# SensorsINI/v2e

Hardware: NVIDIA H100
Metric: Mevents/s (higher is better)
Workload: dtype fp16 tensor-core convs (fp32 accumulate) + f64 pixel state

## Files before the change

include/v2e_b200.h:

```cpp
#ifndef V2E_B200_H
#define V2E_B200_H

#include <stdint.h>

#ifdef __cplusplus
extern "C" {
#endif

typedef enum V2eStatus {
    V2E_OK = 0,
    V2E_E_INVALID = -1,
    V2E_E_CUDA = -2,
    V2E_E_CAPACITY = -3,
    V2E_E_ITER_CAP = -4,
    V2E_E_STATE = -5,
    V2E_E_UNSUPPORTED = -6,
    V2E_E_FALLBACK = -7
} V2eStatus;

typedef enum V2eFrameDtype { V2E_U8 = 0, V2E_F32 = 1, V2E_F64 = 2 } V2eFrameDtype;

const char *v2e_last_error(void);
int v2e_version(void);
int v2e_abi_info(int *version, int *emu_cfg_size, int *frame_info_size, int *unet_weights_size);
// ... 139 lines not shown
int v2e_conv2d_lrelu_sm100(const void *x1_dev, int C1, const void *x2_dev, int C2,
                           const void *wgt_dev, const float *bias_dev, int Cout_pad, int KH, int KW,
                           int N, int H, int W, void *out_dev, int out_cstride, int out_mode,
                           int co_real, float slope, void *stream);

enum {
    V2E_CONV_TILE_AUTO = -1,
    V2E_CONV_TILE_LEGACY = 0,
    V2E_CONV_TILE_256x128 = 1,
    V2E_CONV_TILE_128x256 = 2
};
int v2e_conv2d_lrelu_sm100_tile(const void *x1_dev, int C1, const void *x2_dev, int C2,
                                const void *wgt_dev, const float *bias_dev, int Cout_pad, int KH, int KW,
                                int N, int H, int W, void *out_dev, int out_cstride, int out_mode,
                                int co_real, float slope, int tile, void *stream);
int v2e_conv_pick_tile(int C1, int C2, int Cout_pad, int KH, int KW, int N, int H, int W, int n_sms);

int v2e_conv2d_lrelu_sm100_strip(const void *x1_dev, int C1, const void *x2_dev, int C2,
                                 const void *wgt_row_dev, const float *bias_dev, int Cout_pad, int KH,
                                 int KW, int N, int H, int W, void *out_dev, int out_cstride,
                                 int out_mode, int co_real, float slope, void *stream);
int v2e_conv_strip_pick_kc(int C1, int C2, int Cout_pad, int KH, int KW, int W);

enum {
    V2E_STRIP_CHAIN_AUTO = -1,
    V2E_STRIP_CHAIN_PAIRED = 0,
    V2E_STRIP_CHAIN_STACKED = 1
};
int v2e_conv2d_lrelu_sm100_strip_chain(const void *x1_dev, int C1, const void *x2_dev, int C2,
                                       const void *wgt_row_dev, const float *bias_dev, int Cout_pad, int KH,
// ... 97 lines not shown
```

v2e_b200/_lib.py:

```python
import ctypes
import os

from . import build as _build

_LIB = None


class V2eEmuCfg(ctypes.Structure):
    _fields_ = [
        ("width", ctypes.c_int32), ("height", ctypes.c_int32),
        ("per_pixel_thres", ctypes.c_int32), ("hdr", ctypes.c_int32),
        ("pos_thres_nominal", ctypes.c_double), ("neg_thres_nominal", ctypes.c_double),
        ("cutoff_hz", ctypes.c_double), ("leak_rate_hz", ctypes.c_double),
        ("leak_jitter_fraction", ctypes.c_double), ("refractory_period_s", ctypes.c_double),
        ("shot_noise_rate_hz", ctypes.c_double), ("shot_inten_factor", ctypes.c_double),
        ("rng_mode", ctypes.c_int32), ("iter_cap", ctypes.c_int32),
        ("seed", ctypes.c_uint64),
        ("csdvs", ctypes.c_int32), ("max_frames_per_step", ctypes.c_int32),
        ("cs_tau_p_s", ctypes.c_double), ("cs_tau_h_s", ctypes.c_double),
        ("scidvs", ctypes.c_int32), ("photoreceptor_noise", ctypes.c_int32),
        ("rng_pixel_offset", ctypes.c_uint32), ("full_frame_px", ctypes.c_uint32),
        ("own_row0", ctypes.c_int32), ("own_rows", ctypes.c_int32),
        ("cs_halo_rows", ctypes.c_int32), ("reserved1", ctypes.c_int32),
    ]
# ... 61 lines not shown
    "v2e_emu_cs_pack": (_i, [_vp, _vp]),
    "v2e_emu_cs_unpack_from": (_i, [_vp, _vp, _vp, _vp]),
    "v2e_emu_cs_send_dev": (_vp, [_vp]),
    "v2e_emu_cs_chunk": (_i, [_vp, _i, _i, _vp]),
    "v2e_emu_cs_max_dev": (_vp, [_vp]),
    "v2e_emu_cs_advance": (_i, [_vp, _i, _i, _vp]),
    "v2e_emu_cs_update": (_i, [_vp, _vp, _i, _vp, _vp, _vp]),
    "v2e_emu_phase_filter": (_i, [_vp, _d, _d, _u64, _i, _vp]),
    "v2e_emu_read_counts": (_i, [_vp, ctypes.POINTER(ctypes.c_int32), _vp, _i, _vp]),
    "v2e_emu_phase_shot": (_i, [_vp, _vp, _i, _d, _d, _vp, _u64, _vp]),
    "v2e_emu_phase_emit": (_i, [_vp, _d, _d, _vp, _u64, _vp]),
    "v2e_conv2d_lrelu_sm100": (_i, [_vp, _i, _vp, _i, _vp, _vp, _i, _i, _i, _i, _i, _i, _vp, _i, _i, _i,
                                    ctypes.c_float, _vp]),
    "v2e_conv2d_lrelu_sm100_tile": (_i, [_vp, _i, _vp, _i, _vp, _vp, _i, _i, _i, _i, _i, _i, _vp, _i, _i, _i,
                                         ctypes.c_float, _i, _vp]),
    "v2e_conv_pick_tile": (_i, [_i, _i, _i, _i, _i, _i, _i, _i, _i]),
    "v2e_conv2d_lrelu_sm100_strip": (_i, [_vp, _i, _vp, _i, _vp, _vp, _i, _i, _i, _i, _i, _i, _vp, _i, _i, _i,
                                          ctypes.c_float, _vp]),
    "v2e_conv_strip_pick_kc": (_i, [_i, _i, _i, _i, _i, _i]),
    "v2e_conv2d_lrelu_sm100_strip_chain": (_i, [_vp, _i, _vp, _i, _vp, _vp, _i, _i, _i, _i, _i, _i, _vp, _i, _i, _i,
                                                ctypes.c_float, _i, _vp]),
    "v2e_conv_strip_pick_chain": (_i, [_i, _i, _i, _i, _i, _i]),
    "v2e_conv2d_up2_lrelu_sm100": (_i, [_vp, _i, _vp, _vp, _vp, _i, _i, _i, _i, _vp, _i, ctypes.c_float, _vp]),
    "v2e_conv_up2_fold_weights": (_i, [_vp, _i, _i, _i, _i, _vp]),
    "v2e_conv_up2_supported_c": (_i, [_i, _i, _i]),
    "v2e_slomo_create": (_i, [_i, _i, _i, _vp, _vp, ctypes.POINTER(_vp)]),
    "v2e_slomo_destroy": (_i, [_vp]),
    "v2e_slomo_set_pairs": (_i, [_vp, _vp, _i, _vp]),
    "v2e_slomo_max_flow": (_i, [_vp, ctypes.POINTER(ctypes.c_float), _vp]),
    "v2e_slomo_interp": (_i, [_vp, _d, _vp, _vp, _vp]),
# ... 106 lines not shown
```

v2e_b200/csrc/conv_tc.cu:

```cuda
#include <cuda.h>
#include <cuda_fp16.h>
#include <cuda_runtime.h>
#include <math.h>
#include <stdint.h>
#include <stdio.h>
#include <string.h>
#include <vector>

#include "../../include/v2e_b200.h"
#include "common.cuh"
#include "tc_common.cuh"

namespace {

constexpr int kTileH = 8, kTileW = 16, kBM = kTileH * kTileW;
constexpr int kStages = 4;
constexpr int kConvThreads = 288;
constexpr int kProducerWarp = 8;
constexpr int kConsumerWarps = 8;

struct ConvParams {
    int N, H, W;
    int C1, C2;
    int KH, KW;
    int KC;
    int BN;
    int stages;
    int co_fast;
    int tiles_x, tiles_y;
    int n_tiles;
    int out_cstride;
    int out_mode;
    int co_real;
    float slope;
    const float *bias;
    void *out;
};

__device__ __forceinline__ uint8_t *align1024(uint8_t *p) { return (uint8_t *)(((uintptr_t)p + 1023) & ~(uintptr_t)1023); }

__device__ __forceinline__ float lrelu(float x, float slope) { return x > 0.f ? x : x * slope; }

template <int BN>
__device__ __forceinline__ void epilogue_row(const float (&d)[BN / 2], int i, bool inb, size_t pix, int lane,
                                             const float *bias, float slope, int out_mode, void *out, int cstride,
                                             int co0, __half2 (&h)[BN / 8]) {
#pragma unroll
    for (int j = 0; j < BN / 8; j++) {
        const int c = 8 * j + 2 * (lane & 3);
        const float x0 = lrelu(d[4 * j + 2 * i] + __ldg(bias + c), slope);
        const float x1 = lrelu(d[4 * j + 2 * i + 1] + __ldg(bias + c + 1), slope);
        h[j] = __floats2half2_rn(x0, x1);
        if (inb) {
            if (out_mode == 0) *(__half2 *)((__half *)out + pix * cstride + co0 + c) = h[j];
            else if (j == 0) *(float2 *)((float *)out + pix * 8 + c) = make_float2(x0, x1);
        }
// ... 1 lines not shown
}

template <int BN>
__global__ void __launch_bounds__(kConvThreads, 1)
conv_tc_kernel(const __grid_constant__ CUtensorMap tmA, const __grid_constant__ CUtensorMap tmA2,
               const __grid_constant__ CUtensorMap tmB, const ConvParams p) {
    extern __shared__ __align__(1024) uint8_t smem_raw[];
    uint8_t *smem = align1024(smem_raw);
    const uint32_t a_bytes = kBM * p.KC * 2;
    const uint32_t b_bytes_raw = BN * p.KC * 2;
    const uint32_t b_bytes = (b_bytes_raw + 1023) & ~1023u;
    const uint32_t stage_bytes = a_bytes + b_bytes;
    __shared__ __align__(8) uint64_t full_bar[kStages], empty_bar[kStages];

    const int warp = threadIdx.x >> 5, lane = threadIdx.x & 31;
    const int tile = p.co_fast ? blockIdx.y : blockIdx.x;
    const int tx = tile % p.tiles_x, ty = (tile / p.tiles_x) % p.tiles_y, n = tile / (p.tiles_x * p.tiles_y);
    const int x0 = tx * kTileW, y0 = ty * kTileH;
    const int n0 = (p.co_fast ? blockIdx.x : blockIdx.y) * BN;
    const int Ctot = p.C1 + p.C2;
    const int slabs = Ctot / p.KC;
    const int k_iters = p.KH * p.KW * slabs;

    if (threadIdx.x == 0) {
        for (int s = 0; s < kStages; s++) { mbar_init(&full_bar[s], 1); mbar_init(&empty_bar[s], kConsumerWarps); }
        fence_barrier_init();
    }
    if (warp == kProducerWarp && lane == 0) {
        prefetch_tmap(&tmA);
        if (p.C2) prefetch_tmap(&tmA2);
        prefetch_tmap(&tmB);
    }
    __syncthreads();

    if (warp == kProducerWarp) {
        if (lane == 0) {
            int stage = 0;
            uint32_t phase = 0;
            const int ph = p.KH / 2, pw = p.KW / 2;
            for (int tap = 0; tap < p.KH * p.KW; tap++) {
                const int r = tap / p.KW, s = tap % p.KW;
                for (int sl = 0; sl < slabs; sl++) {
                    mbar_wait(&empty_bar[stage], phase ^ 1);
                    uint8_t *sa = smem + stage * stage_bytes, *sb = sa + a_bytes;
                    mbar_expect_tx(&full_bar[stage], a_bytes + b_bytes_raw);
                    const int c = sl * p.KC;
                    if (c < p.C1) tma_load_4d(sa, &tmA, &full_bar[stage], c, x0 + s - pw, y0 + r - ph, n);
                    else tma_load_4d(sa, &tmA2, &full_bar[stage], c - p.C1, x0 + s - pw, y0 + r - ph, n);
                    tma_load_2d(sb, &tmB, &full_bar[stage], tap * Ctot + c, n0);
                    if (++stage == p.stages) { stage = 0; phase ^= 1; }
                }
            }
        }
    } else {
        const int g = warp >> 2;
        const uint64_t d0 = make_smem_desc(smem_u32(smem), swizzle_layout(p.KC), 8u * p.KC * 2u);
        const uint32_t stage16 = stage_bytes >> 4, a16 = a_bytes >> 4, half16 = (64u * p.KC * 2u) >> 4;
        const int ksteps = p.KC / 16;
        float acc[BN / 2];
#pragma unroll
        for (int i = 0; i < BN / 2; i++) acc[i] = 0.f;
        int stage = 0, prev = -1;
        uint32_t phase = 0;
        for (int it = 0; it < k_iters; it++) {
            mbar_wait(&full_bar[stage], phase);
            const uint32_t base = (uint32_t)stage * stage16;
            wgmma_fence();
            for (int j = 0; j < ksteps; j++)
                wgmma_f16<BN>(acc, desc_add(d0, base + (uint32_t)g * half16 + 2u * j), desc_add(d0, base + a16 + 2u * j),
                              (uint32_t)((it | j) != 0));
            wgmma_commit();
            wgmma_wait<1>();
            if (prev >= 0) { __syncwarp(); if (lane == 0) mbar_arrive(&empty_bar[prev]); }
            prev = stage;
            if (++stage == p.stages) { stage = 0; phase ^= 1; }
        }
        wgmma_wait<0>();
        wgmma_fence_regs(acc);
        __half2 hv[BN / 8];
#pragma unroll
        for (int i = 0; i < 2; i++) {
            const int m = 64 * g + 16 * (warp & 3) + (lane >> 2) + 8 * i;
            const int py = y0 + m / kTileW, px = x0 + m % kTileW;
            const bool inb = py < p.H && px < p.W;
            const size_t pix = ((size_t)n * p.H + py) * p.W + px;
            epilogue_row<BN>(acc, i, inb, pix, lane, p.bias + n0, p.slope, p.out_mode, p.out, p.out_cstride, n0, hv);
        }
    }
}

template <int MH, int BN>
__global__ void __launch_bounds__(kConvThreads, 1)
conv_wide_kernel(const __grid_constant__ CUtensorMap tmA, const __grid_constant__ CUtensorMap tmA2,
                 const __grid_constant__ CUtensorMap tmB, const ConvParams p) {
    constexpr int TH = kTileH * MH, BM = kBM * MH;
    extern __shared__ __align__(1024) uint8_t smem_raw[];
    uint8_t *smem = align1024(smem_raw);
    const uint32_t a_bytes = BM * p.KC * 2;
    const uint32_t b_bytes = BN * p.KC * 2;
    const uint32_t stage_bytes = a_bytes + b_bytes;
    __shared__ __align__(8) uint64_t full_bar[kStages], empty_bar[kStages];

    const int warp = threadIdx.x >> 5, lane = threadIdx.x & 31;
    const int tile = p.co_fast ? blockIdx.y : blockIdx.x;
    const int tx = tile % p.tiles_x, ty = (tile / p.tiles_x) % p.tiles_y, n = tile / (p.tiles_x * p.tiles_y);
    const int x0 = tx * kTileW, y0 = ty * TH;
    const int n0 = (p.co_fast ? blockIdx.x : blockIdx.y) * BN;
    const int Ctot = p.C1 + p.C2;
    const int slabs = Ctot / p.KC;
    const int k_iters = p.KH * p.KW * slabs;

    if (threadIdx.x == 0) {
        for (int s = 0; s < kStages; s++) { mbar_init(&full_bar[s], 1); mbar_init(&empty_bar[s], kConsumerWarps); }
        fence_barrier_init();
    }
    if (warp == kProducerWarp && lane == 0) {
        prefetch_tmap(&tmA);
        if (p.C2) prefetch_tmap(&tmA2);
        prefetch_tmap(&tmB);
    }
    __syncthreads();

    if (warp == kProducerWarp) {
        if (lane == 0) {
            int stage = 0;
            uint32_t phase = 0;
            const int ph = p.KH / 2, pw = p.KW / 2;
            for (int tap = 0; tap < p.KH * p.KW; tap++) {
                const int r = tap / p.KW, s = tap % p.KW;
                for (int sl = 0; sl < slabs; sl++) {
                    mbar_wait(&empty_bar[stage], phase ^ 1);
                    uint8_t *sa = smem + stage * stage_bytes, *sb = sa + a_bytes;
                    mbar_expect_tx(&full_bar[stage], a_bytes + b_bytes);
                    const int c = sl * p.KC;
                    if (c < p.C1) tma_load_4d(sa, &tmA, &full_bar[stage], c, x0 + s - pw, y0 + r - ph, n);
                    else tma_load_4d(sa, &tmA2, &full_bar[stage], c - p.C1, x0 + s - pw, y0 + r - ph, n);
                    tma_load_2d(sb, &tmB, &full_bar[stage], tap * Ctot + c, n0);
                    if (++stage == p.stages) { stage = 0; phase ^= 1; }
                }
            }
        }
    } else {
        const int g = __shfl_sync(0xffffffffu, warp >> 2, 0);
        const uint64_t d0 = make_smem_desc(smem_u32(smem), swizzle_layout(p.KC), 8u * p.KC * 2u);
        const uint32_t stage16 = stage_bytes >> 4, a16 = a_bytes >> 4, q16 = (64u * p.KC * 2u) >> 4;
        const int ksteps = p.KC / 16;
        float acc[MH][BN / 2];
#pragma unroll
        for (int h = 0; h < MH; h++) {
#pragma unroll
            for (int i = 0; i < BN / 2; i++) acc[h][i] = 0.f;
            wgmma_fence_regs(acc[h]);
        }
        int stage = 0, prev = -1;
        uint32_t phase = 0;
        for (int it = 0; it < k_iters; it++) {
            mbar_wait(&full_bar[stage], phase);
            const uint32_t base = (uint32_t)stage * stage16;
            wgmma_fence();
            for (int j = 0; j < ksteps; j++) {
#pragma unroll
                for (int h = 0; h < MH; h++)
                    wgmma_f16<BN>(acc[h], desc_add(d0, base + (uint32_t)(g * MH + h) * q16 + 2u * j),
                                  desc_add(d0, base + a16 + 2u * j), (uint32_t)((it | j) != 0));
            }
            wgmma_commit();
            wgmma_wait<1>();
            if (prev >= 0) { __syncwarp(); if (lane == 0) mbar_arrive(&empty_bar[prev]); }
            prev = stage;
            if (++stage == p.stages) { stage = 0; phase ^= 1; }
        }
        wgmma_wait<0>();
#pragma unroll
        for (int h = 0; h < MH; h++) wgmma_fence_regs(acc[h]);
        const float *bias = p.bias + n0;
        __half *out = (__half *)p.out + n0;
#pragma unroll
        for (int h = 0; h < MH; h++) {
            size_t pix[2];
            bool inb[2];
#pragma unroll
            for (int i = 0; i < 2; i++) {
                const int m = 64 * (g * MH + h) + 16 * (warp & 3) + (lane >> 2) + 8 * i;
                const int py = y0 + m / kTileW, px = x0 + m % kTileW;
                inb[i] = py < p.H && px < p.W;
                pix[i] = (((size_t)n * p.H + py) * p.W + px) * p.out_cstride;
            }
#pragma unroll
            for (int j = 0; j < BN / 8; j++) {
                const int c = 8 * j + 2 * (lane & 3);
                const float2 b = __ldg((const float2 *)(bias + c));
#pragma unroll
                for (int i = 0; i < 2; i++)
                    if (inb[i])
                        *(__half2 *)(out + pix[i] + c) = __floats2half2_rn(lrelu(acc[h][4 * j + 2 * i] + b.x, p.slope),
                                                                           lrelu(acc[h][4 * j + 2 * i + 1] + b.y, p.slope));
            }
        }
    }
}


constexpr int kRowTile = 128;

struct StripParams {
    int N, H, W;
    int C1, C2;
    int KH, KW;
    int KC, BN;
    int tiles_x, seg_h, n_seg, n_items;
    int nslot;
    void *pool_out;
// ... 528 lines not shown
        long tiles = (long)((W + kTileW - 1) / kTileW) * ((H + kTileH * mh - 1) / (kTileH * mh)) * N;
        const long ctas = tiles * (Cout_pad / bn);
        const long waves = (ctas + n_sms - 1) / n_sms;
        const double a_bytes = (double)kBM * mh * kc * 2, b_bytes = (double)bn * kc * 2;
        const double flops = 2.0 * kBM * mh * bn * kc;
        const double per_stage = fmax((a_bytes + b_bytes) / 24.0, flops / 4096.0);
        const double cost = (double)waves * per_stage;
        if (tile == V2E_CONV_TILE_LEGACY || cost < best_cost) { best = tile; best_cost = cost; }
    }
    return best;
}

struct V2eConvLaunch {
    CUtensorMap tmA, tmA2, tmB;
    ConvParams p;
    dim3 grid;
    int mh;
    size_t smem;
};

int v2e_conv_prepare(V2eConvLaunch *L, const void *x1, int C1, const void *x2, int C2, const void *wgt,
                     const float *bias, int Cout_pad, int KH, int KW, int N, int H, int W, void *out,
                     int out_cstride, int out_mode, int co_real, float slope, int tile, int n_sms) {
    if (C1 % 16 || C2 % 16 || !(Cout_pad == 16 || Cout_pad == 32 || Cout_pad == 64 || (Cout_pad > 0 && Cout_pad % 128 == 0)))
        return v2e_set_error(V2E_E_INVALID, "conv: channel counts must be padded to 16 (Cout to 16/32/64/128k)%s", "");
    if (tile == V2E_CONV_TILE_AUTO) tile = v2e_conv_pick_tile(C1, C2, Cout_pad, KH, KW, N, H, W, n_sms);
    if (tile < V2E_CONV_TILE_LEGACY || tile > V2E_CONV_TILE_128x256)
        return v2e_set_error(V2E_E_INVALID, "conv: unknown tile%s", "");
    memset(L, 0, sizeof(*L));
    ConvParams &p = L->p;
    int mh, bn;
    tile_shape(tile, Cout_pad, &mh, &bn);
    const bool wide = tile != V2E_CONV_TILE_LEGACY;
    p.N = N; p.H = H; p.W = W; p.C1 = C1; p.C2 = C2; p.KH = KH; p.KW = KW;
    p.KC = v2e_conv_pick_kc(C1, C2);
    p.BN = bn;
    if (wide && (Cout_pad % bn || out_mode != 0))
        return v2e_set_error(V2E_E_INVALID, "conv: the wide tiles need fp16 output and Cout_pad a multiple of their width%s", "");
    p.stages = kStages;
    p.tiles_x = (W + kTileW - 1) / kTileW;
    p.tiles_y = (H + kTileH * mh - 1) / (kTileH * mh);
    p.n_tiles = p.tiles_x * p.tiles_y * N;
    p.out_cstride = out_cstride; p.out_mode = out_mode; p.co_real = co_real; p.slope = slope;
    p.bias = bias; p.out = out;
    L->mh = mh;
    int rc;
    if ((rc = make_act_tmap_h(&L->tmA, x1, N, H, W, C1, p.KC, kTileH * mh))) return rc;
    if (C2) { if ((rc = make_act_tmap_h(&L->tmA2, x2, N, H, W, C2, p.KC, kTileH * mh))) return rc; }
    else L->tmA2 = L->tmA;
    if ((rc = v2e_make_wgt_tmap(&L->tmB, wgt, Cout_pad, KH * KW * (C1 + C2), p.KC, bn))) return rc;
    const unsigned tiles = (unsigned)p.n_tiles, cob = (unsigned)(Cout_pad / p.BN);
    p.co_fast = (cob > 1 && tiles <= 65535u) ? 1 : 0;
    L->grid = p.co_fast ? dim3(cob, tiles, 1) : dim3(tiles, cob, 1);
    size_t stage = (size_t)kBM * mh * p.KC * 2 + (((size_t)p.BN * p.KC * 2 + 1023) & ~(size_t)1023);
    L->smem = stage * p.stages + 1024;
    return V2E_OK;
}

template <int BN>
static cudaError_t conv_launch_bn(const V2eConvLaunch *L, cudaStream_t st) {
    static PerDeviceOnce attr_once;
    if (attr_once.first()) cudaFuncSetAttribute(conv_tc_kernel<BN>, cudaFuncAttributeMaxDynamicSharedMemorySize, 200 * 1024);
    conv_tc_kernel<BN><<<L->grid, kConvThreads, L->smem, st>>>(L->tmA, L->tmA2, L->tmB, L->p);
    return cudaGetLastError();
}

template <int MH, int BN>
static cudaError_t conv_launch_wide(const V2eConvLaunch *L, cudaStream_t st) {
    static PerDeviceOnce attr_once;
    if (attr_once.first())
        cudaFuncSetAttribute(conv_wide_kernel<MH, BN>, cudaFuncAttributeMaxDynamicSharedMemorySize, 226 * 1024);
    conv_wide_kernel<MH, BN><<<L->grid, kConvThreads, L->smem, st>>>(L->tmA, L->tmA2, L->tmB, L->p);
    return cudaGetLastError();
}

int v2e_conv_launch(const V2eConvLaunch *L, cudaStream_t st) {
    cudaError_t e;
    if (L->mh == 2 && L->p.BN == 128) e = conv_launch_wide<2, 128>(L, st);
    else if (L->mh == 1 && L->p.BN == 256) e = conv_launch_wide<1, 256>(L, st);
    else switch (L->p.BN) {
        case 16: e = conv_launch_bn<16>(L, st); break;
        case 32: e = conv_launch_bn<32>(L, st); break;
        case 64: e = conv_launch_bn<64>(L, st); break;
        case 128: e = conv_launch_bn<128>(L, st); break;
        default: return v2e_set_error(V2E_E_UNSUPPORTED, "conv_tc_kernel: unsupported tile width%s", "");
    }
    if (e != cudaSuccess) return v2e_set_error(V2E_E_CUDA, "conv_tc_kernel launch: %s", cudaGetErrorString(e));
    return V2E_OK;
}

size_t v2e_conv_launch_size(void) { return sizeof(V2eConvLaunch); }

static int device_sms() {
    int dev = 0, sms = 132;
    cudaGetDevice(&dev);
    cudaDeviceGetAttribute(&sms, cudaDevAttrMultiProcessorCount, dev);
    return sms;
}

extern "C" int v2e_conv2d_lrelu_sm100_tile(const void *x1_dev, int C1, const void *x2_dev, int C2,
                                           const void *wgt_dev, const float *bias_dev, int Cout_pad, int KH, int KW,
                                           int N, int H, int W, void *out_dev, int out_cstride, int out_mode,
                                           int co_real, float slope, int tile, void *stream) {
    V2eConvLaunch L;
    int rc = v2e_conv_prepare(&L, x1_dev, C1, x2_dev, C2, wgt_dev, bias_dev, Cout_pad, KH, KW, N, H, W, out_dev,
                              out_cstride, out_mode, co_real, slope, tile, device_sms());
    if (rc) return rc;
    return v2e_conv_launch(&L, (cudaStream_t)stream);
}

extern "C" int v2e_conv2d_lrelu_sm100(const void *x1_dev, int C1, const void *x2_dev, int C2,
                                      const void *wgt_dev, const float *bias_dev, int Cout_pad, int KH, int KW,
                                      int N, int H, int W, void *out_dev, int out_cstride, int out_mode,
                                      int co_real, float slope, void *stream) {
    return v2e_conv2d_lrelu_sm100_tile(x1_dev, C1, x2_dev, C2, wgt_dev, bias_dev, Cout_pad, KH, KW, N, H, W, out_dev,
                                       out_cstride, out_mode, co_real, slope, V2E_CONV_TILE_AUTO, stream);
}

struct V2eStripLaunch {
    CUtensorMap tmA, tmA2, tmB;
    StripParams p;
    int stacked;
    int grid;
// ... 344 lines not shown
```

v2e_b200/csrc/slomo.cu:

```cuda
#include <cuda.h>
#include <cuda_fp16.h>
#include <cuda_runtime.h>
#include <math.h>
#include <stdint.h>
#include <stdio.h>
#include <string.h>

#include <vector>

#include "../../include/v2e_b200.h"
#include "common.cuh"

struct V2eConvLaunch;
int v2e_conv_prepare(V2eConvLaunch *L, const void *x1, int C1, const void *x2, int C2, const void *wgt,
                     const float *bias, int Cout_pad, int KH, int KW, int N, int H, int W, void *out,
                     int out_cstride, int out_mode, int co_real, float slope, int tile, int n_sms);
int v2e_conv_launch(const V2eConvLaunch *L, cudaStream_t st);
size_t v2e_conv_launch_size(void);
struct V2eStripLaunch;
int v2e_strip_pick(int C1, int C2, int Cout_pad, int KH, int KW, int W, int *nslot_out);
size_t v2e_strip_launch_size(void);
int v2e_strip_pool_supported(int C1, int C2, int Cout_pad, int KH, int KW, int H, int W);
int v2e_strip_prepare(V2eStripLaunch *L, const void *x1, int C1, const void *x2, int C2, const void *wgt_row,
                      const float *bias, int Cout_pad, int KH, int KW, int N, int H, int W, void *out,
                      int out_cstride, int out_mode, int co_real, float slope, int n_sms, void *pool_out,
                      int pool_cstride, int chain);
int v2e_strip_launch(const V2eStripLaunch *L, cudaStream_t st);
struct V2eUpLaunch;
int v2e_conv_up2_supported(int C, int Cout_pad, int W_out);
extern "C" int v2e_conv_up2_fold_weights(const float *w, int cout, int cin, int Cout_pad, int C_pad, void *out_host);
size_t v2e_conv_up2_launch_size(void);
// ... 427 lines not shown
static int conv(V2eSlomo *h, const UNet &u, int li, const __half *x1, const __half *x2, int B, int H, int W, void *out,
                int out_mode, cudaStream_t st, __half *pool_out = nullptr) {
    int rc;
    const bool row = u.row_kc[li] != 0;
    V2eConvLaunch *L = (V2eConvLaunch *)h->launch_mem.data();
    V2eStripLaunch *R = (V2eStripLaunch *)h->row_mem.data();
    h->ran[&u == &h->interp][li] = row ? (pool_out ? V2E_SLOMO_KERNEL_STRIP_POOL : V2E_SLOMO_KERNEL_STRIP)
                                       : V2E_SLOMO_KERNEL_TAP;
    if (row)
        rc = v2e_strip_prepare(R, x1, u.c1p[li], x2, x2 ? u.c2p[li] : 0, u.w_row[li], u.b[li], u.cout_pad[li], u.L[li].k,
                               u.L[li].k, B, H, W, out, u.cout_pad[li], out_mode, u.L[li].cout, kSlope, h->n_sms,
                               pool_out, u.cout_pad[li], V2E_STRIP_CHAIN_AUTO);
    else
        rc = v2e_conv_prepare(L, x1, u.c1p[li], x2, x2 ? u.c2p[li] : 0, u.w[li], u.b[li], u.cout_pad[li], u.L[li].k,
                              u.L[li].k, B, H, W, out, u.cout_pad[li], out_mode, u.L[li].cout, kSlope,
                              V2E_CONV_TILE_AUTO, h->n_sms);
    if (rc) return rc;
    if (h->profile) {
        if (h->ev_used + 2 > h->ev.size()) {
            size_t old = h->ev.size();
            h->ev.resize(old + 512);
            for (size_t i = old; i < h->ev.size(); i++) cudaEventCreate(&h->ev[i]);
        }
        cudaEventRecord(h->ev[h->ev_used], st);
    }
    rc = row ? v2e_strip_launch(R, st) : v2e_conv_launch(L, st);
    if (h->profile) {
        cudaEventRecord(h->ev[h->ev_used + 1], st);
        h->ev_used += 2;
        const LayerSpec &l = u.L[li];
        const double fl = 2.0 * B * H * W * (double)l.cout * (l.cin1 + l.cin2) * l.k * l.k;
// ... 20 lines not shown
    }
    rc = v2e_conv_up2_launch(L, st);
    if (h->profile) {
        cudaEventRecord(h->ev[h->ev_used + 1], st);
        h->ev_used += 2;
        const LayerSpec &l = u.L[li];
        const double fl = 2.0 * B * H * W * (double)l.cout * l.cin1 * 9;
        h->conv_flops += fl;
        h->ev_layer.push_back(li);
        h->ev_flops.push_back(fl);
    }
    return rc;
}

static bool pool_fusable(const V2eSlomo *h, const UNet &u, int li, int H, int W) {
    if (h->no_fused_pool || !u.row_kc[li] || u.cout_pad[li] != u.L[li].cout) return false;
    return v2e_strip_pool_supported(u.c1p[li], u.c2p[li], u.cout_pad[li], u.L[li].k, u.L[li].k, H, W) != 0;
}

static int unet_forward(V2eSlomo *h, const UNet &u, const __half *in, float *out, int B, cudaStream_t st) {
    const int H = h->H, W = h->W;
    int rc;
    if ((rc = conv(h, u, 0, in, nullptr, B, H, W, h->x0, 0, st))) return rc;
    bool pooled = pool_fusable(h, u, 1, H, W);
    if ((rc = conv(h, u, 1, h->x0, nullptr, B, H, W, h->s1, 0, st, pooled ? h->pool[0] : nullptr))) return rc;
    const int ch[6] = {32, 64, 128, 256, 512, 512};
    const __half *prev = h->s1;
    for (int l = 0; l < 5; l++) {
        const int hi = H >> l, wi = W >> l, ho = hi / 2, wo = wi / 2;
        if (!pooled) {
            const long n = (long)B * ho * wo * (ch[l] / 8);
// ... 233 lines not shown
```

v2e_b200/csrc/tc_common.cuh:

```cuda
#pragma once
#include <cuda.h>
#include <cuda_runtime.h>
#include <stdint.h>

__device__ __forceinline__ uint32_t smem_u32(const void *p) { return (uint32_t)__cvta_generic_to_shared(p); }

__device__ __forceinline__ void mbar_init(uint64_t *bar, uint32_t count) {
    asm volatile("mbarrier.init.shared::cta.b64 [%0], %1;" ::"r"(smem_u32(bar)), "r"(count) : "memory");
}
__device__ __forceinline__ void fence_barrier_init() { asm volatile("fence.mbarrier_init.release.cluster;" ::: "memory"); }
__device__ __forceinline__ void fence_proxy_async() { asm volatile("fence.proxy.async.shared::cta;" ::: "memory"); }
__device__ __forceinline__ void mbar_expect_tx(uint64_t *bar, uint32_t bytes) {
    asm volatile("mbarrier.arrive.expect_tx.shared::cta.b64 _, [%0], %1;" ::"r"(smem_u32(bar)), "r"(bytes) : "memory");
}
__device__ __forceinline__ void mbar_arrive(uint64_t *bar) {
    asm volatile("mbarrier.arrive.shared::cta.b64 _, [%0];" ::"r"(smem_u32(bar)) : "memory");
}
__device__ __forceinline__ void mbar_wait(uint64_t *bar, uint32_t parity) {
    const uint32_t addr = smem_u32(bar);
    uint32_t done;
    do {
        asm volatile(
            "{\n\t.reg .pred p;\n\t"
            "mbarrier.try_wait.parity.shared::cta.b64 p, [%1], %2;\n\t"
// ... 3 lines not shown
}

__device__ __forceinline__ void prefetch_tmap(const CUtensorMap *tm) {
    asm volatile("prefetch.tensormap [%0];" ::"l"((uint64_t)tm) : "memory");
}
__device__ __forceinline__ void tma_load_4d(void *dst, const CUtensorMap *tm, uint64_t *bar, int c0, int c1, int c2, int c3) {
    asm volatile(
        "cp.async.bulk.tensor.4d.shared::cluster.global.tile.mbarrier::complete_tx::bytes [%0], [%1, {%3, %4, %5, %6}], [%2];"
        ::"r"(smem_u32(dst)), "l"((uint64_t)tm), "r"(smem_u32(bar)), "r"(c0), "r"(c1), "r"(c2), "r"(c3) : "memory");
}
__device__ __forceinline__ void tma_load_2d(void *dst, const CUtensorMap *tm, uint64_t *bar, int c0, int c1) {
    asm volatile(
        "cp.async.bulk.tensor.2d.shared::cluster.global.tile.mbarrier::complete_tx::bytes [%0], [%1, {%3, %4}], [%2];"
        ::"r"(smem_u32(dst)), "l"((uint64_t)tm), "r"(smem_u32(bar)), "r"(c0), "r"(c1) : "memory");
}

__device__ __forceinline__ uint32_t elect_one() {
    uint32_t pred;
    asm volatile("{\n\t.reg .pred p;\n\telect.sync _|p, 0xffffffff;\n\tselp.u32 %0, 1, 0, p;\n\t}" : "=r"(pred));
    return pred;
}

__device__ __forceinline__ void wgmma_fence() { asm volatile("wgmma.fence.sync.aligned;" ::: "memory"); }
__device__ __forceinline__ void wgmma_commit() { asm volatile("wgmma.commit_group.sync.aligned;" ::: "memory"); }
template <int N>
__device__ __forceinline__ void wgmma_wait() { asm volatile("wgmma.wait_group.sync.aligned %0;" ::"n"(N) : "memory"); }
template <int R>
__device__ __forceinline__ void wgmma_fence_regs(float (&d)[R]) {
#pragma unroll
    for (int i = 0; i < R; i++) asm volatile("" : "+f"(d[i])::"memory");
// ... 57 lines not shown
```

Baseline: 57.38.

## Make implicit-GEMM conv kernels persistent and fuse avg-pool into epilogue

Turns the tensor-core conv kernels into persistent kernels. A grid sized from occupancy times the SM count loops over (tile, cout-block) items. The TMA/mbarrier pipeline carries its stage counter across items, so the next tile's loads overlap the current epilogue. The wide kernel gets an extra producer warpgroup (384 threads) with setmaxnreg redistribution to give consumers more registers. A fused 2x2 average-pool epilogue reads back the written output and removes a separate pool kernel for non-strip layers. Risks include serialised epilogues inside each CTA, extra global re-reads for the pool, and a per-item load imbalance tail.

```diff
diff --git a/include/v2e_b200.h b/include/v2e_b200.h
--- a/include/v2e_b200.h
+++ b/include/v2e_b200.h
@@ -177,6 +177,10 @@
                                 const void *wgt_dev, const float *bias_dev, int Cout_pad, int KH, int KW,
                                 int N, int H, int W, void *out_dev, int out_cstride, int out_mode,
                                 int co_real, float slope, int tile, void *stream);
+int v2e_conv2d_lrelu_sm100_plan(const void *x1_dev, int C1, const void *x2_dev, int C2,
+                                const void *wgt_dev, const float *bias_dev, int Cout_pad, int KH, int KW,
+                                int N, int H, int W, void *out_dev, int out_cstride, int out_mode,
+                                int co_real, float slope, int tile, int n_sms, void *pool_out_dev, void *stream);
 int v2e_conv_pick_tile(int C1, int C2, int Cout_pad, int KH, int KW, int N, int H, int W, int n_sms);
 
 int v2e_conv2d_lrelu_sm100_strip(const void *x1_dev, int C1, const void *x2_dev, int C2,
diff --git a/v2e_b200/_lib.py b/v2e_b200/_lib.py
--- a/v2e_b200/_lib.py
+++ b/v2e_b200/_lib.py
@@ -99,6 +99,8 @@
                                     ctypes.c_float, _vp]),
     "v2e_conv2d_lrelu_sm100_tile": (_i, [_vp, _i, _vp, _i, _vp, _vp, _i, _i, _i, _i, _i, _i, _vp, _i, _i, _i,
                                          ctypes.c_float, _i, _vp]),
+    "v2e_conv2d_lrelu_sm100_plan": (_i, [_vp, _i, _vp, _i, _vp, _vp, _i, _i, _i, _i, _i, _i, _vp, _i, _i, _i,
+                                         ctypes.c_float, _i, _i, _vp, _vp]),
     "v2e_conv_pick_tile": (_i, [_i, _i, _i, _i, _i, _i, _i, _i, _i]),
     "v2e_conv2d_lrelu_sm100_strip": (_i, [_vp, _i, _vp, _i, _vp, _vp, _i, _i, _i, _i, _i, _i, _vp, _i, _i, _i,
                                           ctypes.c_float, _vp]),
diff --git a/v2e_b200/csrc/conv_tc.cu b/v2e_b200/csrc/conv_tc.cu
--- a/v2e_b200/csrc/conv_tc.cu
+++ b/v2e_b200/csrc/conv_tc.cu
@@ -17,6 +17,8 @@
 constexpr int kStages = 4;
 constexpr int kConvThreads = 288;
 constexpr int kProducerWarp = 8;
+constexpr int kWideThreads = 384;
+constexpr int kWideProducerRegs = 40, kWideConsumerRegs = 232;
 constexpr int kConsumerWarps = 8;
 
 struct ConvParams {
@@ -25,21 +27,82 @@
     int KH, KW;
     int KC;
     int BN;
-    int stages;
-    int co_fast;
     int tiles_x, tiles_y;
-    int n_tiles;
+    int cob;
+    int n_items;
     int out_cstride;
     int out_mode;
     int co_real;
     float slope;
     const float *bias;
     void *out;
+    void *pool_out;
+    int pool_cstride;
 };
 
 __device__ __forceinline__ uint8_t *align1024(uint8_t *p) { return (uint8_t *)(((uintptr_t)p + 1023) & ~(uintptr_t)1023); }
 
 __device__ __forceinline__ float lrelu(float x, float slope) { return x > 0.f ? x : x * slope; }
+
+__device__ __forceinline__ void tap_item(const ConvParams &p, int w, int TH, int &n, int &x0, int &y0, int &n0) {
+    const int tile = w / p.cob;
+    n0 = (w - tile * p.cob) * p.BN;
+    const int tx = tile % p.tiles_x, ty = (tile / p.tiles_x) % p.tiles_y;
+    n = tile / (p.tiles_x * p.tiles_y);
+    x0 = tx * kTileW;
+    y0 = ty * TH;
+}
+
+__device__ __forceinline__ void tap_produce(const ConvParams &p, const CUtensorMap *tmA, const CUtensorMap *tmA2,
+                                            const CUtensorMap *tmB, uint8_t *smem, uint64_t *full_bar,
+                                            uint64_t *empty_bar, int TH, uint32_t a_bytes, uint32_t b_bytes,
+                                            uint32_t tx_bytes) {
+    const uint32_t stage_bytes = a_bytes + b_bytes;
+    const int Ctot = p.C1 + p.C2, slabs = Ctot / p.KC;
+    const int ph = p.KH / 2, pw = p.KW / 2;
+    uint32_t q = 0;
+    for (int w = blockIdx.x; w < p.n_items; w += gridDim.x) {
+        int n, x0, y0, n0;
+        tap_item(p, w, TH, n, x0, y0, n0);
+        for (int tap = 0; tap < p.KH * p.KW; tap++) {
+            const int r = tap / p.KW, s = tap % p.KW;
+            for (int sl = 0; sl < slabs; sl++, q++) {
+                const uint32_t stage = q % kStages;
+                mbar_wait(&empty_bar[stage], ((q / kStages) & 1u) ^ 1u);
+                uint8_t *sa = smem + stage * stage_bytes, *sb = sa + a_bytes;
+                mbar_expect_tx(&full_bar[stage], tx_bytes);
+                const int c = sl * p.KC;
+                if (c < p.C1) tma_load_4d(sa, tmA, &full_bar[stage], c, x0 + s - pw, y0 + r - ph, n);
+                else tma_load_4d(sa, tmA2, &full_bar[stage], c - p.C1, x0 + s - pw, y0 + r - ph, n);
+                tma_load_2d(sb, tmB, &full_bar[stage], tap * Ctot + c, n0);
+            }
+        }
+    }
+}
+
+__device__ __forceinline__ void tap_pool(const ConvParams &p, int g, int rows, int n, int x0, int y0, int n0) {
+    asm volatile("bar.sync %0, 128;" ::"r"(1 + g) : "memory");
+    const int Ho = p.H / 2, Wo = p.W / 2, c8n = p.BN / 8;
+    const int oy0 = (y0 + rows * g) / 2, ox0 = x0 / 2, total = rows / 2 * (kTileW / 2) * c8n;
+    const size_t cs = (size_t)p.out_cstride, rs = (size_t)p.W * cs;
+    for (int e = threadIdx.x & 127; e < total; e += 128) {
+        const int c8 = e % c8n, r = e / c8n;
+        const int ox = ox0 + r % (kTileW / 2), oy = oy0 + r / (kTileW / 2);
+        if (oy >= Ho || ox >= Wo) continue;
+        const __half *s = (const __half *)p.out + (((size_t)n * p.H + 2 * oy) * p.W + 2 * ox) * cs + n0 + c8 * 8;
+        uint4 a = __ldcg((const uint4 *)s), b = __ldcg((const uint4 *)(s + cs)), c = __ldcg((const uint4 *)(s + rs)),
+              d = __ldcg((const uint4 *)(s + rs + cs));
+        const __half2 *ha = (const __half2 *)&a, *hb = (const __half2 *)&b, *hc = (const __half2 *)&c, *hd = (const __half2 *)&d;
+        uint4 o;
+        __half2 *ho = (__half2 *)&o;
+#pragma unroll
+        for (int j = 0; j < 4; j++) {
+            float2 fa = __half22float2(ha[j]), fb = __half22float2(hb[j]), fc = __half22float2(hc[j]), fd = __half22float2(hd[j]);
+            ho[j] = __floats2half2_rn((fa.x + fb.x + fc.x + fd.x) * 0.25f, (fa.y + fb.y + fc.y + fd.y) * 0.25f);
+        }
+        *(uint4 *)((__half *)p.pool_out + (((size_t)n * Ho + oy) * Wo + ox) * p.pool_cstride + n0 + c8 * 8) = o;
+    }
+}
 
 template <int BN>
 __device__ __forceinline__ void epilogue_row(const float (&d)[BN / 2], int i, bool inb, size_t pix, int lane,
@@ -71,13 +134,7 @@
     __shared__ __align__(8) uint64_t full_bar[kStages], empty_bar[kStages];
 
     const int warp = threadIdx.x >> 5, lane = threadIdx.x & 31;
-    const int tile = p.co_fast ? blockIdx.y : blockIdx.x;
-    const int tx = tile % p.tiles_x, ty = (tile / p.tiles_x) % p.tiles_y, n = tile / (p.tiles_x * p.tiles_y);
-    const int x0 = tx * kTileW, y0 = ty * kTileH;
-    const int n0 = (p.co_fast ? blockIdx.x : blockIdx.y) * BN;
-    const int Ctot = p.C1 + p.C2;
-    const int slabs = Ctot / p.KC;
-    const int k_iters = p.KH * p.KW * slabs;
+    const int k_iters = p.KH * p.KW * ((p.C1 + p.C2) / p.KC);
 
     if (threadIdx.x == 0) {
         for (int s = 0; s < kStages; s++) { mbar_init(&full_bar[s], 1); mbar_init(&empty_bar[s], kConsumerWarps); }
@@ -91,63 +148,51 @@
     __syncthreads();
 
     if (warp == kProducerWarp) {
-        if (lane == 0) {
-            int stage = 0;
-            uint32_t phase = 0;
-            const int ph = p.KH / 2, pw = p.KW / 2;
-            for (int tap = 0; tap < p.KH * p.KW; tap++) {
-                const int r = tap / p.KW, s = tap % p.KW;
-                for (int sl = 0; sl < slabs; sl++) {
-                    mbar_wait(&empty_bar[stage], phase ^ 1);
-                    uint8_t *sa = smem + stage * stage_bytes, *sb = sa + a_bytes;
-                    mbar_expect_tx(&full_bar[stage], a_bytes + b_bytes_raw);
-                    const int c = sl * p.KC;
-                    if (c < p.C1) tma_load_4d(sa, &tmA, &full_bar[stage], c, x0 + s - pw, y0 + r - ph, n);
-                    else tma_load_4d(sa, &tmA2, &full_bar[stage], c - p.C1, x0 + s - pw, y0 + r - ph, n);
-                    tma_load_2d(sb, &tmB, &full_bar[stage], tap * Ctot + c, n0);
-                    if (++stage == p.stages) { stage = 0; phase ^= 1; }
-                }
-            }
-        }
+        if (lane == 0) tap_produce(p, &tmA, &tmA2, &tmB, smem, full_bar, empty_bar, kTileH, a_bytes, b_bytes,
+                                   a_bytes + b_bytes_raw);
     } else {
         const int g = warp >> 2;
         const uint64_t d0 = make_smem_desc(smem_u32(smem), swizzle_layout(p.KC), 8u * p.KC * 2u);
         const uint32_t stage16 = stage_bytes >> 4, a16 = a_bytes >> 4, half16 = (64u * p.KC * 2u) >> 4;
         const int ksteps = p.KC / 16;
-        float acc[BN / 2];
-#pragma unroll
-        for (int i = 0; i < BN / 2; i++) acc[i] = 0.f;
-        int stage = 0, prev = -1;
-        uint32_t phase = 0;
-        for (int it = 0; it < k_iters; it++) {
-            mbar_wait(&full_bar[stage], phase);
-            const uint32_t base = (uint32_t)stage * stage16;
-            wgmma_fence();
-            for (int j = 0; j < ksteps; j++)
-                wgmma_f16<BN>(acc, desc_add(d0, base + (uint32_t)g * half16 + 2u * j), desc_add(d0, base + a16 + 2u * j),
-                              (uint32_t)((it | j) != 0));
-            wgmma_commit();
-            wgmma_wait<1>();
-            if (prev >= 0) { __syncwarp(); if (lane == 0) mbar_arrive(&empty_bar[prev]); }
-            prev = stage;
-            if (++stage == p.stages) { stage = 0; phase ^= 1; }
+        uint32_t q = 0;
+        for (int w = blockIdx.x; w < p.n_items; w += gridDim.x) {
+            float acc[BN / 2];
+#pragma unroll
+            for (int i = 0; i < BN / 2; i++) acc[i] = 0.f;
+            for (int it = 0; it < k_iters; it++, q++) {
+                mbar_wait(&full_bar[q % kStages], (q / kStages) & 1u);
+                const uint32_t base = (q % kStages) * stage16;
+                wgmma_fence();
+                for (int j = 0; j < ksteps; j++)
+                    wgmma_f16<BN>(acc, desc_add(d0, base + (uint32_t)g * half16 + 2u * j),
+                                  desc_add(d0, base + a16 + 2u * j), (uint32_t)((it | j) != 0));
+                wgmma_commit();
+                wgmma_wait<1>();
+                if (it > 0) { __syncwarp(); if (lane == 0) mbar_arrive(&empty_bar[(q - 1) % kStages]); }
+            }
+            wgmma_wait<0>();
+            __syncwarp();
+            if (lane == 0) mbar_arrive(&empty_bar[(q - 1) % kStages]);
+            int n, x0, y0, n0;
+            tap_item(p, w, kTileH, n, x0, y0, n0);
+            wgmma_fence_regs(acc);
+            __half2 hv[BN / 8];
+#pragma unroll
+            for (int i = 0; i < 2; i++) {
+                const int m = 64 * g + 16 * (warp & 3) + (lane >> 2) + 8 * i;
+                const int py = y0 + m / kTileW, px = x0 + m % kTileW;
+                const bool inb = py < p.H && px < p.W;
+                const size_t pix = ((size_t)n * p.H + py) * p.W + px;
+                epilogue_row<BN>(acc, i, inb, pix, lane, p.bias + n0, p.slope, p.out_mode, p.out, p.out_cstride, n0, hv);
+            }
+            if (p.pool_out) tap_pool(p, g, kTileH / 2, n, x0, y0, n0);
         }
-        wgmma_wait<0>();
-        wgmma_fence_regs(acc);
-        __half2 hv[BN / 8];
-#pragma unroll
-        for (int i = 0; i < 2; i++) {
-            const int m = 64 * g + 16 * (warp & 3) + (lane >> 2) + 8 * i;
-            const int py = y0 + m / kTileW, px = x0 + m % kTileW;
-            const bool inb = py < p.H && px < p.W;
-            const size_t pix = ((size_t)n * p.H + py) * p.W + px;
-            epilogue_row<BN>(acc, i, inb, pix, lane, p.bias + n0, p.slope, p.out_mode, p.out, p.out_cstride, n0, hv);
-        }
     }
 }
 
 template <int MH, int BN>
-__global__ void __launch_bounds__(kConvThreads, 1)
+__global__ void __launch_bounds__(kWideThreads, 1)
 conv_wide_kernel(const __grid_constant__ CUtensorMap tmA, const __grid_constant__ CUtensorMap tmA2,
                  const __grid_constant__ CUtensorMap tmB, const ConvParams p) {
     constexpr int TH = kTileH * MH, BM = kBM * MH;
@@ -159,13 +204,7 @@
     __shared__ __align__(8) uint64_t full_bar[kStages], empty_bar[kStages];
 
     const int warp = threadIdx.x >> 5, lane = threadIdx.x & 31;
-    const int tile = p.co_fast ? blockIdx.y : blockIdx.x;
-    const int tx = tile % p.tiles_x, ty = (tile / p.tiles_x) % p.tiles_y, n = tile / (p.tiles_x * p.tiles_y);
-    const int x0 = tx * kTileW, y0 = ty * TH;
-    const int n0 = (p.co_fast ? blockIdx.x : blockIdx.y) * BN;
-    const int Ctot = p.C1 + p.C2;
-    const int slabs = Ctot / p.KC;
-    const int k_iters = p.KH * p.KW * slabs;
+    const int k_iters = p.KH * p.KW * ((p.C1 + p.C2) / p.KC);
 
     if (threadIdx.x == 0) {
         for (int s = 0; s < kStages; s++) { mbar_init(&full_bar[s], 1); mbar_init(&empty_bar[s], kConsumerWarps); }
@@ -178,81 +217,71 @@
     }
     __syncthreads();
 
-    if (warp == kProducerWarp) {
-        if (lane == 0) {
-            int stage = 0;
-            uint32_t phase = 0;
-            const int ph = p.KH / 2, pw = p.KW / 2;
-            for (int tap = 0; tap < p.KH * p.KW; tap++) {
-                const int r = tap / p.KW, s = tap % p.KW;
-                for (int sl = 0; sl < slabs; sl++) {
-                    mbar_wait(&empty_bar[stage], phase ^ 1);
-                    uint8_t *sa = smem + stage * stage_bytes, *sb = sa + a_bytes;
-                    mbar_expect_tx(&full_bar[stage], a_bytes + b_bytes);
-                    const int c = sl * p.KC;
-                    if (c < p.C1) tma_load_4d(sa, &tmA, &full_bar[stage], c, x0 + s - pw, y0 + r - ph, n);
-                    else tma_load_4d(sa, &tmA2, &full_bar[stage], c - p.C1, x0 + s - pw, y0 + r - ph, n);
-                    tma_load_2d(sb, &tmB, &full_bar[stage], tap * Ctot + c, n0);
-                    if (++stage == p.stages) { stage = 0; phase ^= 1; }
-                }
-            }
-        }
+    if (warp >= kProducerWarp) {
+        setmaxnreg_dec<kWideProducerRegs>();
+        if (warp == kProducerWarp && lane == 0)
+            tap_produce(p, &tmA, &tmA2, &tmB, smem, full_bar, empty_bar, TH, a_bytes, b_bytes, a_bytes + b_bytes);
     } else {
+        setmaxnreg_inc<kWideConsumerRegs>();
         const int g = __shfl_sync(0xffffffffu, warp >> 2, 0);
         const uint64_t d0 = make_smem_desc(smem_u32(smem), swizzle_layout(p.KC), 8u * p.KC * 2u);
         const uint32_t stage16 = stage_bytes >> 4, a16 = a_bytes >> 4, q16 = (64u * p.KC * 2u) >> 4;
         const int ksteps = p.KC / 16;
-        float acc[MH][BN / 2];
-#pragma unroll
-        for (int h = 0; h < MH; h++) {
-#pragma unroll
-            for (int i = 0; i < BN / 2; i++) acc[h][i] = 0.f;
-            wgmma_fence_regs(acc[h]);
-        }
-        int stage = 0, prev = -1;
-        uint32_t phase = 0;
-        for (int it = 0; it < k_iters; it++) {
-            mbar_wait(&full_bar[stage], phase);
-            const uint32_t base = (uint32_t)stage * stage16;
-            wgmma_fence();
-            for (int j = 0; j < ksteps; j++) {
-#pragma unroll
-                for (int h = 0; h < MH; h++)
-                    wgmma_f16<BN>(acc[h], desc_add(d0, base + (uint32_t)(g * MH + h) * q16 + 2u * j),
-                                  desc_add(d0, base + a16 + 2u * j), (uint32_t)((it | j) != 0));
-            }
-            wgmma_commit();
-            wgmma_wait<1>();
-            if (prev >= 0) { __syncwarp(); if (lane == 0) mbar_arrive(&empty_bar[prev]); }
-            prev = stage;
-            if (++stage == p.stages) { stage = 0; phase ^= 1; }
-        }
-        wgmma_wait<0>();
-#pragma unroll
-        for (int h = 0; h < MH; h++) wgmma_fence_regs(acc[h]);
-        const float *bias = p.bias + n0;
-        __half *out = (__half *)p.out + n0;
-#pragma unroll
-        for (int h = 0; h < MH; h++) {
-            size_t pix[2];
-            bool inb[2];
-#pragma unroll
-            for (int i = 0; i < 2; i++) {
-                const int m = 64 * (g * MH + h) + 16 * (warp & 3) + (lane >> 2) + 8 * i;
-                const int py = y0 + m / kTileW, px = x0 + m % kTileW;
-                inb[i] = py < p.H && px < p.W;
-                pix[i] = (((size_t)n * p.H + py) * p.W + px) * p.out_cstride;
-            }
-#pragma unroll
-            for (int j = 0; j < BN / 8; j++) {
-                const int c = 8 * j + 2 * (lane & 3);
-                const float2 b = __ldg((const float2 *)(bias + c));
-#pragma unroll
-                for (int i = 0; i < 2; i++)
-                    if (inb[i])
-                        *(__half2 *)(out + pix[i] + c) = __floats2half2_rn(lrelu(acc[h][4 * j + 2 * i] + b.x, p.slope),
-                                                                           lrelu(acc[h][4 * j + 2 * i + 1] + b.y, p.slope));
-            }
+        uint32_t q = 0;
+        for (int w = blockIdx.x; w < p.n_items; w += gridDim.x) {
+            float acc[MH][BN / 2];
+#pragma unroll
+            for (int h = 0; h < MH; h++) {
+#pragma unroll
+                for (int i = 0; i < BN / 2; i++) acc[h][i] = 0.f;
+                wgmma_fence_regs(acc[h]);
+            }
+            for (int it = 0; it < k_iters; it++, q++) {
+                mbar_wait(&full_bar[q % kStages], (q / kStages) & 1u);
+                const uint32_t base = (q % kStages) * stage16;
+                wgmma_fence();
+                for (int j = 0; j < ksteps; j++) {
+#pragma unroll
+                    for (int h = 0; h < MH; h++)
+                        wgmma_f16<BN>(acc[h], desc_add(d0, base + (uint32_t)(g * MH + h) * q16 + 2u * j),
+                                      desc_add(d0, base + a16 + 2u * j), (uint32_t)((it | j) != 0));
+                }
+                wgmma_commit();
+                wgmma_wait<1>();
+                if (it > 0) { __syncwarp(); if (lane == 0) mbar_arrive(&empty_bar[(q - 1) % kStages]); }
+            }
+            wgmma_wait<0>();
+            __syncwarp();
+            if (lane == 0) mbar_arrive(&empty_bar[(q - 1) % kStages]);
+            int n, x0, y0, n0;
+            tap_item(p, w, TH, n, x0, y0, n0);
+#pragma unroll
+            for (int h = 0; h < MH; h++) wgmma_fence_regs(acc[h]);
+            const float *bias = p.bias + n0;
+            __half *out = (__half *)p.out + n0;
+#pragma unroll
+            for (int h = 0; h < MH; h++) {
+                size_t pix[2];
+                bool inb[2];
+#pragma unroll
+                for (int i = 0; i < 2; i++) {
+                    const int m = 64 * (g * MH + h) + 16 * (warp & 3) + (lane >> 2) + 8 * i;
+                    const int py = y0 + m / kTileW, px = x0 + m % kTileW;
+                    inb[i] = py < p.H && px < p.W;
+                    pix[i] = (((size_t)n * p.H + py) * p.W + px) * p.out_cstride;
+                }
+#pragma unroll
+                for (int j = 0; j < BN / 8; j++) {
+                    const int c = 8 * j + 2 * (lane & 3);
+                    const float2 b = __ldg((const float2 *)(bias + c));
+#pragma unroll
+                    for (int i = 0; i < 2; i++)
+                        if (inb[i])
+                            *(__half2 *)(out + pix[i] + c) = __floats2half2_rn(lrelu(acc[h][4 * j + 2 * i] + b.x, p.slope),
+                                                                               lrelu(acc[h][4 * j + 2 * i + 1] + b.y, p.slope));
+                }
+            }
+            if (p.pool_out) tap_pool(p, g, TH / 2, n, x0, y0, n0);
         }
     }
 }
@@ -811,14 +840,30 @@
 struct V2eConvLaunch {
     CUtensorMap tmA, tmA2, tmB;
     ConvParams p;
-    dim3 grid;
-    int mh;
+    const void *fn;
+    unsigned grid, threads;
     size_t smem;
 };
 
+static const void *tap_kernel(int mh, int bn) {
+    static PerDeviceOnce once[6];
+    const void *fn;
+    int k, lim = 200 * 1024;
+    if (mh == 2 && bn == 128) { fn = (const void *)conv_wide_kernel<2, 128>; k = 0; lim = 226 * 1024; }
+    else if (mh == 1 && bn == 256) { fn = (const void *)conv_wide_kernel<1, 256>; k = 1; lim = 226 * 1024; }
+    else if (mh == 1 && bn == 16) { fn = (const void *)conv_tc_kernel<16>; k = 2; }
+    else if (mh == 1 && bn == 32) { fn = (const void *)conv_tc_kernel<32>; k = 3; }
+    else if (mh == 1 && bn == 64) { fn = (const void *)conv_tc_kernel<64>; k = 4; }
+    else if (mh == 1 && bn == 128) { fn = (const void *)conv_tc_kernel<128>; k = 5; }
+    else return nullptr;
+    if (once[k].first()) cudaFuncSetAttribute(fn, cudaFuncAttributeMaxDynamicSharedMemorySize, lim);
+    return fn;
+}
+
 int v2e_conv_prepare(V2eConvLaunch *L, const void *x1, int C1, const void *x2, int C2, const void *wgt,
                      const float *bias, int Cout_pad, int KH, int KW, int N, int H, int W, void *out,
-                     int out_cstride, int out_mode, int co_real, float slope, int tile, int n_sms) {
+                     int out_cstride, int out_mode, int co_real, float slope, int tile, int n_sms, void *pool_out,
+                     int pool_cstride) {
     if (C1 % 16 || C2 % 16 || !(Cout_pad == 16 || Cout_pad == 32 || Cout_pad == 64 || (Cout_pad > 0 && Cout_pad % 128 == 0)))
         return v2e_set_error(V2E_E_INVALID, "conv: channel counts must be padded to 16 (Cout to 16/32/64/128k)%s", "");
     if (tile == V2E_CONV_TILE_AUTO) tile = v2e_conv_pick_tile(C1, C2, Cout_pad, KH, KW, N, H, W, n_sms);
@@ -834,54 +879,38 @@
     p.BN = bn;
     if (wide && (Cout_pad % bn || out_mode != 0))
         return v2e_set_error(V2E_E_INVALID, "conv: the wide tiles need fp16 output and Cout_pad a multiple of their width%s", "");
-    p.stages = kStages;
     p.tiles_x = (W + kTileW - 1) / kTileW;
     p.tiles_y = (H + kTileH * mh - 1) / (kTileH * mh);
-    p.n_tiles = p.tiles_x * p.tiles_y * N;
+    p.cob = Cout_pad / p.BN;
+    const long items = (long)p.tiles_x * p.tiles_y * N * p.cob;
+    if (items > 0x7fffffffL) return v2e_set_error(V2E_E_INVALID, "conv: too many output tiles%s", "");
+    p.n_items = (int)items;
     p.out_cstride = out_cstride; p.out_mode = out_mode; p.co_real = co_real; p.slope = slope;
     p.bias = bias; p.out = out;
-    L->mh = mh;
+    if (pool_out && (out_mode != 0 || H % 2 || W % 2 || pool_cstride < Cout_pad))
+        return v2e_set_error(V2E_E_INVALID, "conv: the pooled epilogue needs fp16 output and even H, W%s", "");
+    p.pool_out = pool_out; p.pool_cstride = pool_cstride;
+    if (!(L->fn = tap_kernel(mh, bn))) return v2e_set_error(V2E_E_UNSUPPORTED, "conv_tc_kernel: unsupported tile width%s", "");
     int rc;
     if ((rc = make_act_tmap_h(&L->tmA, x1, N, H, W, C1, p.KC, kTileH * mh))) return rc;
     if (C2) { if ((rc = make_act_tmap_h(&L->tmA2, x2, N, H, W, C2, p.KC, kTileH * mh))) return rc; }
     else L->tmA2 = L->tmA;
     if ((rc = v2e_make_wgt_tmap(&L->tmB, wgt, Cout_pad, KH * KW * (C1 + C2), p.KC, bn))) return rc;
-    const unsigned tiles = (unsigned)p.n_tiles, cob = (unsigned)(Cout_pad / p.BN);
-    p.co_fast = (cob > 1 && tiles <= 65535u) ? 1 : 0;
-    L->grid = p.co_fast ? dim3(cob, tiles, 1) : dim3(tiles, cob, 1);
     size_t stage = (size_t)kBM * mh * p.KC * 2 + (((size_t)p.BN * p.KC * 2 + 1023) & ~(size_t)1023);
-    L->smem = stage * p.stages + 1024;
+    L->smem = stage * kStages + 1024;
+    int per_sm = 1;
+    L->threads = wide ? kWideThreads : kConvThreads;
+    cudaError_t e = cudaOccupancyMaxActiveBlocksPerMultiprocessor(&per_sm, L->fn, L->threads, L->smem);
+    if (e != cudaSuccess) return v2e_set_error(V2E_E_CUDA, "conv_tc_kernel occupancy: %s", cudaGetErrorString(e));
+    if (per_sm < 1) per_sm = 1;
+    const long ctas = (long)per_sm * (n_sms < 1 ? 1 : n_sms);
+    L->grid = (unsigned)(ctas < items ? ctas : items);
     return V2E_OK;
 }
 
-template <int BN>
-static cudaError_t conv_launch_bn(const V2eConvLaunch *L, cudaStream_t st) {
-    static PerDeviceOnce attr_once;
-    if (attr_once.first()) cudaFuncSetAttribute(conv_tc_kernel<BN>, cudaFuncAttributeMaxDynamicSharedMemorySize, 200 * 1024);
-    conv_tc_kernel<BN><<<L->grid, kConvThreads, L->smem, st>>>(L->tmA, L->tmA2, L->tmB, L->p);
-    return cudaGetLastError();
-}
-
-template <int MH, int BN>
-static cudaError_t conv_launch_wide(const V2eConvLaunch *L, cudaStream_t st) {
-    static PerDeviceOnce attr_once;
-    if (attr_once.first())
-        cudaFuncSetAttribute(conv_wide_kernel<MH, BN>, cudaFuncAttributeMaxDynamicSharedMemorySize, 226 * 1024);
-    conv_wide_kernel<MH, BN><<<L->grid, kConvThreads, L->smem, st>>>(L->tmA, L->tmA2, L->tmB, L->p);
-    return cudaGetLastError();
-}
-
 int v2e_conv_launch(const V2eConvLaunch *L, cudaStream_t st) {
-    cudaError_t e;
-    if (L->mh == 2 && L->p.BN == 128) e = conv_launch_wide<2, 128>(L, st);
-    else if (L->mh == 1 && L->p.BN == 256) e = conv_launch_wide<1, 256>(L, st);
-    else switch (L->p.BN) {
-        case 16: e = conv_launch_bn<16>(L, st); break;
-        case 32: e = conv_launch_bn<32>(L, st); break;
-        case 64: e = conv_launch_bn<64>(L, st); break;
-        case 128: e = conv_launch_bn<128>(L, st); break;
-        default: return v2e_set_error(V2E_E_UNSUPPORTED, "conv_tc_kernel: unsupported tile width%s", "");
-    }
+    void *args[4] = {(void *)&L->tmA, (void *)&L->tmA2, (void *)&L->tmB, (void *)&L->p};
+    cudaError_t e = cudaLaunchKernel(L->fn, dim3(L->grid), dim3(L->threads), args, L->smem, st);
     if (e != cudaSuccess) return v2e_set_error(V2E_E_CUDA, "conv_tc_kernel launch: %s", cudaGetErrorString(e));
     return V2E_OK;
 }
@@ -895,15 +924,24 @@
     return sms;
 }
 
+extern "C" int v2e_conv2d_lrelu_sm100_plan(const void *x1_dev, int C1, const void *x2_dev, int C2,
+                                           const void *wgt_dev, const float *bias_dev, int Cout_pad, int KH, int KW,
+                                           int N, int H, int W, void *out_dev, int out_cstride, int out_mode,
+                                           int co_real, float slope, int tile, int n_sms, void *pool_out_dev,
+                                           void *stream) {
+    V2eConvLaunch L;
+    int rc = v2e_conv_prepare(&L, x1_dev, C1, x2_dev, C2, wgt_dev, bias_dev, Cout_pad, KH, KW, N, H, W, out_dev,
+                              out_cstride, out_mode, co_real, slope, tile, n_sms, pool_out_dev, Cout_pad);
+    if (rc) return rc;
+    return v2e_conv_launch(&L, (cudaStream_t)stream);
+}
+
 extern "C" int v2e_conv2d_lrelu_sm100_tile(const void *x1_dev, int C1, const void *x2_dev, int C2,
                                            const void *wgt_dev, const float *bias_dev, int Cout_pad, int KH, int KW,
                                            int N, int H, int W, void *out_dev, int out_cstride, int out_mode,
                                            int co_real, float slope, int tile, void *stream) {
-    V2eConvLaunch L;
-    int rc = v2e_conv_prepare(&L, x1_dev, C1, x2_dev, C2, wgt_dev, bias_dev, Cout_pad, KH, KW, N, H, W, out_dev,
-                              out_cstride, out_mode, co_real, slope, tile, device_sms());
-    if (rc) return rc;
-    return v2e_conv_launch(&L, (cudaStream_t)stream);
+    return v2e_conv2d_lrelu_sm100_plan(x1_dev, C1, x2_dev, C2, wgt_dev, bias_dev, Cout_pad, KH, KW, N, H, W, out_dev,
+                                       out_cstride, out_mode, co_real, slope, tile, device_sms(), nullptr, stream);
 }
 
 extern "C" int v2e_conv2d_lrelu_sm100(const void *x1_dev, int C1, const void *x2_dev, int C2,
diff --git a/v2e_b200/csrc/slomo.cu b/v2e_b200/csrc/slomo.cu
--- a/v2e_b200/csrc/slomo.cu
+++ b/v2e_b200/csrc/slomo.cu
@@ -14,7 +14,8 @@
 struct V2eConvLaunch;
 int v2e_conv_prepare(V2eConvLaunch *L, const void *x1, int C1, const void *x2, int C2, const void *wgt,
                      const float *bias, int Cout_pad, int KH, int KW, int N, int H, int W, void *out,
-                     int out_cstride, int out_mode, int co_real, float slope, int tile, int n_sms);
+                     int out_cstride, int out_mode, int co_real, float slope, int tile, int n_sms, void *pool_out,
+                     int pool_cstride);
 int v2e_conv_launch(const V2eConvLaunch *L, cudaStream_t st);
 size_t v2e_conv_launch_size(void);
 struct V2eStripLaunch;
@@ -472,7 +473,7 @@
     else
         rc = v2e_conv_prepare(L, x1, u.c1p[li], x2, x2 ? u.c2p[li] : 0, u.w[li], u.b[li], u.cout_pad[li], u.L[li].k,
                               u.L[li].k, B, H, W, out, u.cout_pad[li], out_mode, u.L[li].cout, kSlope,
-                              V2E_CONV_TILE_AUTO, h->n_sms);
+                              V2E_CONV_TILE_AUTO, h->n_sms, pool_out, u.cout_pad[li]);
     if (rc) return rc;
     if (h->profile) {
         if (h->ev_used + 2 > h->ev.size()) {
@@ -523,7 +524,8 @@
 }
 
 static bool pool_fusable(const V2eSlomo *h, const UNet &u, int li, int H, int W) {
-    if (h->no_fused_pool || !u.row_kc[li] || u.cout_pad[li] != u.L[li].cout) return false;
+    if (h->no_fused_pool || u.cout_pad[li] != u.L[li].cout) return false;
+    if (!u.row_kc[li]) return H % 2 == 0 && W % 2 == 0;
     return v2e_strip_pool_supported(u.c1p[li], u.c2p[li], u.cout_pad[li], u.L[li].k, u.L[li].k, H, W) != 0;
 }
 
diff --git a/v2e_b200/csrc/tc_common.cuh b/v2e_b200/csrc/tc_common.cuh
--- a/v2e_b200/csrc/tc_common.cuh
+++ b/v2e_b200/csrc/tc_common.cuh
@@ -41,6 +41,11 @@
         "cp.async.bulk.tensor.2d.shared::cluster.global.tile.mbarrier::complete_tx::bytes [%0], [%1, {%3, %4}], [%2];"
         ::"r"(smem_u32(dst)), "l"((uint64_t)tm), "r"(smem_u32(bar)), "r"(c0), "r"(c1) : "memory");
 }
+
+template <int R>
+__device__ __forceinline__ void setmaxnreg_inc() { asm volatile("setmaxnreg.inc.sync.aligned.u32 %0;" ::"n"(R)); }
+template <int R>
+__device__ __forceinline__ void setmaxnreg_dec() { asm volatile("setmaxnreg.dec.sync.aligned.u32 %0;" ::"n"(R)); }
 
 __device__ __forceinline__ uint32_t elect_one() {
     uint32_t pred;
```

Measured after the change: 58.11 (median of 6 runs). 1.01x the previous value.
